# google/dynamic-video-depth

Hardware: AMD Instinct MI355X
Metric: train iters/s (depth+sceneflow step) at 384x672, 48 pairs; warp+loss HBM GB/s (higher is better)
Workload: dtype f32 (storage and accumulation fp32; conv / MLP contractions on v_mfma_f32_32x32x16_f16: every fp32 operand, scaled by a power of two from its tensor's max, is split into two fp16 terms (22 bits) and a product is three partial products; <= 4e-6 of max|y| against float64, the bound the 3-term bf16 / 6

## Files before the change

dynamic-video-depth_amd/dvd_hip/_lib.py:

```python
import ctypes
import os
import threading

from . import build as _build

c_float_p = ctypes.c_void_p
c_size_t = ctypes.c_size_t
c_int = ctypes.c_int
c_float = ctypes.c_float
c_void_p = ctypes.c_void_p

DVD_OK, DVD_EINVAL, DVD_EHIP, DVD_ENOSPC = 0, -1, -2, -3
ABI_VERSION = 8


class Cameras(ctypes.Structure):
    _fields_ = [(n, c_void_p) for n in ('R_1', 'R_2', 'R_1_T', 'R_2_T', 't_1', 't_2', 'K', 'K_inv')]


class WarpCfg(ctypes.Structure):
    _fields_ = [('B', c_int), ('H', c_int), ('W', c_int), ('midas_mask', c_int), ('crit_l2', c_int),
                ('disp_mode', c_int), ('loss_on_sf', c_int), ('flow_mul', c_float), ('disp_mul', c_float)]


# ... 161 lines not shown
    'dvd_gscale_end': (c_int, [c_void_p, c_void_p]),
    'dvd_cast_scale_f32': (c_int, [c_void_p, c_int, c_void_p, c_longlong, c_void_p, c_void_p]),
    'dvd_maxpool3s2_fwd': (c_int, [c_void_p, c_void_p, c_int, c_void_p, c_longlong, c_int, c_int, c_void_p]),
    'dvd_maxpool3s2_bwd': (c_int, [c_void_p, c_int, c_void_p, c_void_p, c_void_p, c_longlong, c_int, c_int, c_void_p]),
    'dvd_adam_step_guarded': (c_int, [c_void_p, c_void_p, c_float, c_void_p, c_void_p, c_void_p, c_void_p, c_longlong, c_float,
                                      c_float, c_float, c_float, c_int, c_void_p, c_void_p]),
    'dvd_sgd_step': (c_int, [c_void_p, c_void_p, c_float, c_void_p, c_void_p, c_void_p, c_longlong, c_float, c_float, c_float,
                             c_float, c_int, c_void_p]),
    'dvd_sgd_step_guarded': (c_int, [c_void_p, c_void_p, c_float, c_void_p, c_void_p, c_void_p, c_longlong, c_float, c_float,
                                     c_float, c_float, c_int, c_void_p, c_void_p]),
    'dvd_gather_pairs': (c_int, [ctypes.POINTER(GatherItem), c_int, c_void_p, c_int, c_void_p]),
    'dvd_store_gather': (c_int, [ctypes.POINTER(StoreItem), c_int, c_void_p, c_longlong, c_int, c_void_p]),
    'dvd_union_gather': (c_int, [c_void_p] * 5 + [c_int, c_int, c_longlong, c_void_p]),
    'dvd_union_scatter': (c_int, [c_void_p] * 5 + [c_int, c_int, c_longlong, c_void_p]),
    'dvd_union_reduce': (c_int, [c_void_p] * 5 + [c_int, c_int, c_longlong, c_void_p]),
}

_lock = threading.Lock()
_lib = None


def library_path():
    return os.environ.get('DVD_HIP_LIB') or _build.lib_path()


def load():
    global _lib
    if _lib is not None:
        return _lib
    import torch
# ... 29 lines not shown
```

dynamic-video-depth_amd/dvd_hip/conv.py:

```python
import ctypes
import os as _os
import weakref

import torch
import torch.nn.functional as F
from torch import nn

from . import _lib
from .ops import _p, _stream, _workspace, amax_of, chansum, known_amax, new_scalar, set_amax

AB = {k: False for k in ('gconv32', 'no_xwgrad3', 'no_alias', 'no_maskfuse', 'no_s2', 'rowsum')}
for _k in filter(None, _os.environ.get('DVD_AB', '').split(',')):
    if _k not in AB:
        raise RuntimeError('DVD_AB: unknown switch %r (known: %s)' % (_k, ', '.join(sorted(AB))))
    AB[_k] = True


ACT_DTYPES = (torch.float32, torch.float16)
GRAD_SCALE = {'state': None}


def set_grad_scale_state(state):
    GRAD_SCALE['state'] = state

# ... 948 lines not shown
        _lib.check(getattr(lib, family + '_h')(_p(x), _p(gy), _p(_gs(1)), *tail), family + '_h')
    elif family == 'dvd_xwgrad':
        _lib.check(lib.dvd_xwgrad(_p(x), _p(gy), *tail), family)
    elif family == 'dvd_xwgrad1s':
        _lib.check(lib.dvd_xwgrad1s_rowsum(_p(x), _p(x_amax), _p(gy), _p(g_amax), _p(gw), _p(rowsum), *tail[1:]),
                   'dvd_xwgrad1s_rowsum')
    else:
        _lib.check(getattr(lib, family)(_p(x), _p(x_amax), _p(gy), _p(g_amax), *tail), family)
    return gw


class _XConvBn(torch.autograd.Function):

    @staticmethod
    def forward(ctx, x, x_amax, weight, cbias, gamma, beta, mean, var, eps, residual, relu, groups, alias=False, in_site=None,
                out_site=None):
        ctx.set_materialize_grads(False)
        ctx.in_site = in_site if (in_site is not None and not AB['no_maskfuse']) else None
        ctx.out_site = out_site if relu else None
        x = x.contiguous()
        if residual is not None:
            residual = residual.contiguous()
        Cout, _, KS, _ = weight.shape
        y_amax, amax_slot = _fwd_amax(ctx, x)
        y = _xconv_run(x, xconv_packed(weight, False, groups), Cout, KS, bias=cbias, residual=residual, relu_out=relu,
                       groups=groups, bn=(gamma, beta, mean, var, eps), x_amax=x_amax, y_amax=amax_slot)
        ctx.save_for_backward(x, y if relu else None, gamma, mean, var, cbias, x_amax)
        ctx.wparam = weight
        ctx.cfg = (float(eps), bool(relu), residual is not None, groups)
        if alias:
            return y, y_amax, x
        return y, y_amax

    @staticmethod
    def backward(ctx, gy, _g_amax, g_alias=None):
        x, y, gamma, mean, var, cbias, x_amax = ctx.saved_tensors
        weight = ctx.wparam
        eps, relu, has_res, groups = ctx.cfg
        if gy is None:
            return (g_alias,) + (None,) * 14
        gy = gy.contiguous()
        Cout, Cing, KS, _ = weight.shape
        N, _, H, W = gy.shape
        need = ctx.needs_input_grad
        lib = _lib.load()
        dbeta = torch.empty(Cout, device=gy.device, dtype=torch.float32)
        premasked = relu and ctx.out_site is not None and ctx.out_site.is_exactly(gy) and not AB['no_maskfuse']
        mask = relu and not premasked
        need_w = need[2] or (gamma is not None and need[4]) or (cbias is not None and need[3])
        grouped3 = KS == 3 and groups > 1
        wgrad_sums = (relu and need_w and gy.dtype == torch.float32 and (grouped3 or wgrad_reports_rowsum(weight.shape, groups)) and
                      lib.dvd_xwgrad_rowsum_in_kernel(N, Cing * groups, Cout, H, W, KS, groups) == 1)
        no_pass = premasked and wgrad_sums and ctx.out_site.amax is not None
        if relu:
            STATS['sites_no_pass' if (no_pass and AB['rowsum']) else ('sites_premasked' if premasked else 'sites_masked')] += 1
        g = torch.empty_like(gy) if mask else gy
        h16 = _is16(gy)
        if no_pass:
            g_amax = ctx.out_site.amax
        else:
            ws = _workspace(lib.dvd_bnrelu_bwd_workspace_bytes(N, Cout, H * W), gy.device)
            g_amax = _gs(3) if h16 else new_scalar(gy.device)
            _lib.check(lib.dvd_bnrelu_bwd_t(_p(gy), _p(y) if mask else None, None, _p(var), _p(mean), _p(var), eps, None,
                                            _p(g) if mask else None, None, None if wgrad_sums else _p(dbeta), _p(ws),
                                            ctypes.c_size_t(ws.numel()),
                                            int(h16), _p(_gs(1)) if h16 else None, N, Cout, H * W, int(mask), _p(g_amax),
                                            _stream()), 'dvd_bnrelu_bwd')
        gx = gw = gcb = gg = None
        if need[0]:
            gx = _xconv_bwd_data(ctx, g, g_amax, weight, groups, x if ctx.in_site is not None else None, g_alias,
                                 bn_scale=(gamma, var, eps))
        elif g_alias is not None:
            gx = g_alias
        if need_w:
            if wgrad_sums and grouped3:
                gw = xconv_wgrad3_rowsum(x, g, weight.shape, groups, x_amax, g_amax, dbeta)
            else:
                gw = xconv_wgrad(x, g, weight.shape, False, groups, x_amax=x_amax, g_amax=g_amax, rowsum=dbeta if wgrad_sums else None)
            gg = torch.empty_like(gamma) if gamma is not None else None
            gcb = torch.empty_like(cbias) if cbias is not None else None
            _lib.check(lib.dvd_convbn_finalize(_p(weight.detach()), _p(gw), _p(dbeta), _p(gamma), _p(mean), _p(var), eps,
                                               _p(cbias), Cout, Cing * KS * KS, _p(gg), _p(gcb), _stream()),
                       'dvd_convbn_finalize')
        return (gx, None, gw, gcb, gg, (dbeta if need[5] else None), None, None, None, (g if has_res else None), None, None, None,
                None, None)


def conv_bn_act(conv, bn, x, residual=None, relu=True, alias=False):
    if x.is_cuda and x.dtype in ACT_DTYPES and not bn.training and bn.track_running_stats and isinstance(conv, nn.Conv2d):
        xin = None
        if xconv_supported(conv, x):
            xin = x
        elif xconv_strided_1x1_supported(conv, x):
            xin = _subsample(x, conv.stride[0])
        if xin is not None:
            gamma, beta = (bn.weight, bn.bias) if bn.affine else (None, None)
            x_amax = None if _is16(xin) else amax_of(xin)
            in_site = getattr(xin, '_dvd_site', None)
            out_site = _Site() if relu else None
            out = _XConvBn.apply(xin, x_amax, conv.weight, conv.bias, gamma, beta, bn.running_mean, bn.running_var, bn.eps,
                                 residual, relu, conv.groups, bool(alias and xin is x and not AB['no_alias']), in_site, out_site)
            out[0]._dvd_site = out_site
            y = set_amax(out[0], out[1])
            if len(out) == 3:
                return y, set_amax(out[2], x_amax)
            return (y, x) if alias else y
    y = bn_eval_relu(bn, conv(x), residual=residual, relu=relu)
    return (y, x) if alias else y


def xconv_supported(conv, x):
    k = conv.kernel_size
    return (x.is_cuda and x.dtype in ACT_DTYPES and conv.weight.dtype == torch.float32 and
            (conv.groups == 1 or (k[0] == 3 and conv.in_channels // conv.groups >= 32)) and
            k[0] == k[1] and k[0] % 2 == 1 and k[0] <= 11 and tuple(conv.stride) == (1, 1) and
            tuple(conv.dilation) == (1, 1) and tuple(conv.padding) == (k[0] // 2, k[0] // 2) and
            conv.padding_mode == 'zeros')


def xconv_strided_1x1_supported(conv, x):
    return (x.is_cuda and x.dtype in ACT_DTYPES and conv.weight.dtype == torch.float32 and conv.kernel_size == (1, 1) and
# ... 34 lines not shown
```

dynamic-video-depth_amd/dvd_hip/csrc/gconv.hip:

```cpp

#include "dvd_io.h"

namespace dvd {

constexpr int kCPG = 8;
constexpr int kWT_H = 8;

template <bool TRANSPOSED, class T, int TW, int TH>
__global__ __launch_bounds__(256) void gconv3x3_c8_kernel(const T* __restrict__ in, const float* __restrict__ w,
                                                          T* __restrict__ out, int C, int H, int W, int tiles_x) {
  typedef float v2f __attribute__((ext_vector_type(2)));
  typedef float v4f __attribute__((ext_vector_type(4)));
  constexpr int IW = TW + 2 + 2;
  constexpr int IH = TH + 2;
  constexpr int NSX = TW / 4;
  static_assert(TW % 4 == 0 && NSX * TH <= 256, "one thread per strip");
  __shared__ __attribute__((aligned(16))) float s_in[kCPG][IH][IW];
  const int tile = blockIdx.x, g = blockIdx.y, n = blockIdx.z;
  const int ty = tile / tiles_x, tx = tile - ty * tiles_x;
  const int x0 = tx * TW, y0 = ty * TH;
  const size_t plane = (size_t)H * W;
  const T* inb = in + ((size_t)n * C + (size_t)g * kCPG) * plane;
  T* outb = out + ((size_t)n * C + (size_t)g * kCPG) * plane;
  if ((W & 3) == 0) {
    constexpr int kQ = kCPG * IH * NSX, kU = (kQ + 255) / 256;
    float4 v[kU];
#pragma unroll
    for (int u = 0; u < kU; ++u) {
      const int i = threadIdx.x + u * 256;
      const int row = i / NSX, q = i - row * NSX, c = row / IH, yy = row - c * IH;
      const int gy = y0 + yy - 1, gx = x0 + q * 4;
      v[u] = (i < kQ && gy >= 0 && gy < H && gx < W) ? ld4(inb + (size_t)c * plane + (size_t)gy * W + gx)
                                                      : make_float4(0.0f, 0.0f, 0.0f, 0.0f);
    }
    constexpr int kE = kCPG * IH * 2, kUE = (kE + 255) / 256;
    float e[kUE];
#pragma unroll
    for (int u = 0; u < kUE; ++u) {
      const int i = threadIdx.x + u * 256;
      const int row = i >> 1, c = row / IH, yy = row - c * IH;
      const int gy = y0 + yy - 1, gx = (i & 1) ? x0 + TW : x0 - 1;
      e[u] = (i < kE && gy >= 0 && gy < H && gx >= 0 && gx < W) ? ldf(inb + (size_t)c * plane + (size_t)gy * W + gx) : 0.0f;
    }
#pragma unroll
    for (int u = 0; u < kU; ++u) {
      const int i = threadIdx.x + u * 256;
      if (i < kQ) {
        const int row = i / NSX, q = i - row * NSX;
        float* d = &s_in[0][0][0] + row * IW + 1 + q * 4;
        d[0] = v[u].x; d[1] = v[u].y; d[2] = v[u].z; d[3] = v[u].w;
      }
    }
#pragma unroll
    for (int u = 0; u < kUE; ++u) {
      const int i = threadIdx.x + u * 256;
      if (i < kE) (&s_in[0][0][0])[(i >> 1) * IW + ((i & 1) ? TW + 1 : 0)] = e[u];
    }
  } else {
    constexpr int kU = 8, kRow = TW + 2, kTot = kCPG * IH * kRow;
    for (int i0 = threadIdx.x; i0 < kTot; i0 += 256 * kU) {
      float v[kU];
#pragma unroll
      for (int u = 0; u < kU; ++u) {
        const int i = i0 + u * 256;
        const int c = i / (IH * kRow), r = i - c * (IH * kRow), yy = r / kRow, xx = r - yy * kRow;
        const int gy = y0 + yy - 1, gx = x0 + xx - 1;
        v[u] = (i < kTot && gy >= 0 && gy < H && gx >= 0 && gx < W) ? ldf(inb + (size_t)c * plane + (size_t)gy * W + gx) : 0.0f;
      }
#pragma unroll
      for (int u = 0; u < kU; ++u) {
        const int i = i0 + u * 256;
        if (i < kTot) {
          const int c = i / (IH * kRow), r = i - c * (IH * kRow), yy = r / kRow, xx = r - yy * kRow;
          s_in[c][yy][xx] = v[u];
        }
      }
    }
  }
  __syncthreads();
  if (threadIdx.x >= NSX * TH) return;
  const int sy = threadIdx.x / NSX, sx = threadIdx.x - sy * NSX;
  v2f acc[kCPG][2];
#pragma unroll
  for (int d = 0; d < kCPG; ++d) acc[d][0] = acc[d][1] = (v2f){0.0f, 0.0f};
  const float* wg = w + (size_t)g * (kCPG * kCPG * 9);
#pragma unroll 1
  for (int s = 0; s < kCPG; ++s) {
#pragma unroll
    for (int ky = 0; ky < 3; ++ky) {
      const float* row = &s_in[s][sy + ky][sx * 4];
      const v4f a = *reinterpret_cast<const v4f*>(row);
      const v2f b = *reinterpret_cast<const v2f*>(row + 4);
      const v2f xp[3][2] = {{{a.x, a.y}, {a.z, a.w}}, {{a.y, a.z}, {a.w, b.x}}, {{a.z, a.w}, {b.x, b.y}}};
#pragma unroll
      for (int kx = 0; kx < 3; ++kx) {
#pragma unroll
        for (int d = 0; d < kCPG; ++d) {
          const float wv = !TRANSPOSED ? wg[(d * kCPG + s) * 9 + ky * 3 + kx] : wg[(s * kCPG + d) * 9 + (2 - ky) * 3 + (2 - kx)];
          acc[d][0] = __builtin_elementwise_fma(xp[kx][0], (v2f){wv, wv}, acc[d][0]);
          acc[d][1] = __builtin_elementwise_fma(xp[kx][1], (v2f){wv, wv}, acc[d][1]);
        }
      }
    }
  }
  const int oy = y0 + sy, ox = x0 + sx * 4;
  if (oy < H && ox < W) {
    const bool vec = ((W & 3) == 0) && (ox + 3 < W);
#pragma unroll
    for (int d = 0; d < kCPG; ++d) {
      T* dst = outb + (size_t)d * plane + (size_t)oy * W + ox;
      const float o[4] = {acc[d][0].x, acc[d][0].y, acc[d][1].x, acc[d][1].y};
      if (vec) {
        st4(dst, make_float4(o[0], o[1], o[2], o[3]));
      } else {
#pragma unroll
        for (int j = 0; j < 4; ++j)
          if (ox + j < W) stf(dst + j, o[j]);
      }
    }
  }
}

template <bool TRANSPOSED>
static void launch_c8(const void* in, const float* w, void* out, int f16, int N, int C, int H, int W, hipStream_t stream) {
  if (W % 84 == 0) {
    const int tx = W / 84, ty = (H + 11) / 12;
    DVD_DISPATCH_T(f16, hipLaunchKernelGGL((gconv3x3_c8_kernel<TRANSPOSED, T, 84, 12>), dim3(tx * ty, C / kCPG, N), dim3(256), 0,
                                           stream, static_cast<const T*>(in), w, static_cast<T*>(out), C, H, W, tx));
  } else {
    const int tx = (W + 63) / 64, ty = (H + 15) / 16;
    DVD_DISPATCH_T(f16, hipLaunchKernelGGL((gconv3x3_c8_kernel<TRANSPOSED, T, 64, 16>), dim3(tx * ty, C / kCPG, N), dim3(256), 0,
                                           stream, static_cast<const T*>(in), w, static_cast<T*>(out), C, H, W, tx));
  }
}

template <class T, int TW>
__global__ __launch_bounds__(256) void gconv3x3_c8_wgrad_kernel(const T* __restrict__ x, const T* __restrict__ gy,
                                                                float* __restrict__ partial, int C, int H, int W,
                                                                int tiles_x, int G) {
  typedef float v2f __attribute__((ext_vector_type(2)));
  typedef float v4f __attribute__((ext_vector_type(4)));
  constexpr int IW = 68;
  constexpr int IH = kWT_H + 2;
  constexpr int XP = IH * IW + 4;
  constexpr int GW2 = 144;
  constexpr int GP2 = kWT_H * GW2 + 4;
  constexpr int kRedBytes = kWT_H * 32 * 18 * 4, kXBytes = kCPG * XP * 4;
  __shared__ __attribute__((aligned(16))) float s_x[(kRedBytes > kXBytes ? kRedBytes : kXBytes) / 4];
  __shared__ __attribute__((aligned(16))) float s_g[(kCPG / 2) * GP2];
  const int band = blockIdx.x, g = blockIdx.y, n = blockIdx.z;
  const int y0 = band * kWT_H;
  const size_t plane = (size_t)H * W;
  const T* xb = x + ((size_t)n * C + (size_t)g * kCPG) * plane;
  const T* gb = gy + ((size_t)n * C + (size_t)g * kCPG) * plane;
  const bool vec = (W & 3) == 0;

  constexpr int NQ = TW / 4;
  constexpr int kXQ = kCPG * IH * NQ, kUX = (kXQ + 255) / 256;
  constexpr int kXE = kCPG * IH * 2;
  constexpr int kGQ = (kCPG / 2) * kWT_H * NQ, kUG = (kGQ + 255) / 256;
  float4 xv[kUX], g0[kUG], g1[kUG];
  float xe;
  auto fetch = [&](int x0) {
    const float4 z = make_float4(0.0f, 0.0f, 0.0f, 0.0f);
#pragma unroll
    for (int u = 0; u < kUX; ++u) {
      const int i = threadIdx.x + u * 256;
      const int row = i / NQ, q = i - row * NQ, c = row / IH, yy = row - c * IH;
      const int py = y0 + yy - 1, px = x0 + q * 4;
      xv[u] = (i < kXQ && py >= 0 && py < H && px < W) ? ld4(xb + (size_t)c * plane + (size_t)py * W + px) : z;
    }
    {
      const int i = threadIdx.x, row = i >> 1, c = row / IH, yy = row - c * IH;
      const int py = y0 + yy - 1, px = (i & 1) ? x0 + TW : x0 - 1;
      xe = (i < kXE && py >= 0 && py < H && px >= 0 && px < W) ? ldf(xb + (size_t)c * plane + (size_t)py * W + px) : 0.0f;
    }
#pragma unroll
// ... 17 lines not shown
        d[0] = xv[u].x; d[1] = xv[u].y; d[2] = xv[u].z; d[3] = xv[u].w;
      }
    }
    if (threadIdx.x < kXE) {
      const int row = threadIdx.x >> 1, c = row / IH, yy = row - c * IH;
      s_x[c * XP + yy * IW + ((threadIdx.x & 1) ? TW + 1 : 0)] = xe;
    }
#pragma unroll
    for (int u = 0; u < kUG; ++u) {
      const int i = threadIdx.x + u * 256;
      if (i < kGQ) {
        const int row = i / NQ, q = i - row * NQ, cp = row / kWT_H, yy = row - cp * kWT_H;
        v4f* d = reinterpret_cast<v4f*>(&s_g[cp * GP2 + yy * GW2 + q * 8]);
        d[0] = (v4f){g0[u].x, g1[u].x, g0[u].y, g1[u].y};
        d[1] = (v4f){g0[u].z, g1[u].z, g0[u].w, g1[u].w};
      }
    }
  };
  auto stage_scalar = [&](int x0) {
    constexpr int kU = 8, kRow = TW + 2, kTot = kCPG * IH * kRow;
    for (int i0 = threadIdx.x; i0 < kTot; i0 += 256 * kU) {
      float v[kU];
#pragma unroll
      for (int u = 0; u < kU; ++u) {
        const int i = i0 + u * 256;
        const int c = i / (IH * kRow), r = i - c * (IH * kRow), yy = r / kRow, xx = r - yy * kRow;
        const int py = y0 + yy - 1, px = x0 + xx - 1;
        v[u] = (i < kTot && py >= 0 && py < H && px >= 0 && px < W) ? ldf(xb + (size_t)c * plane + (size_t)py * W + px) : 0.0f;
      }
#pragma unroll
// ... 9 lines not shown
    for (int i0 = threadIdx.x; i0 < kTotG; i0 += 256 * kU) {
      float v[kU];
#pragma unroll
      for (int u = 0; u < kU; ++u) {
        const int i = i0 + u * 256;
        const int c = i / (kWT_H * TW), r = i - c * (kWT_H * TW), yy = r / TW, xx = r - yy * TW;
        const int py = y0 + yy, px = x0 + xx;
        v[u] = (i < kTotG && py < H && px < W) ? ldf(gb + (size_t)c * plane + (size_t)py * W + px) : 0.0f;
      }
#pragma unroll
      for (int u = 0; u < kU; ++u) {
        const int i = i0 + u * 256;
        if (i < kTotG) {
          const int c = i / (kWT_H * TW), r = i - c * (kWT_H * TW), yy = r / TW, xx = r - yy * TW;
          s_g[(c >> 1) * GP2 + yy * GW2 + xx * 2 + (c & 1)] = v[u];
        }
      }
    }
  };

  const int lane = threadIdx.x & 63, wave = threadIdx.x >> 6;
  const int r = wave * 2 + (lane >> 5), cp = (lane >> 3) & 3, ci = lane & 7;
  v2f acc[9];
#pragma unroll
  for (int t = 0; t < 9; ++t) acc[t] = (v2f){0.0f, 0.0f};
  const float* grow = &s_g[cp * GP2 + r * GW2];
  const float* xrow = &s_x[ci * XP + r * IW];
  if (vec) fetch(0);
  for (int tx = 0; tx < tiles_x; ++tx) {
    if (vec) put(); else stage_scalar(tx * TW);
// ... 20 lines not shown
    __syncthreads();
  }
  float* s_red = s_x;
#pragma unroll
  for (int t = 0; t < 9; ++t) *reinterpret_cast<v2f*>(&s_red[((r * 32 + cp * 8 + ci) * 9 + t) * 2]) = acc[t];
  __syncthreads();
  float* dst = partial + ((size_t)(n * gridDim.x + band) * G + g) * 576;
  for (int i = threadIdx.x; i < 576; i += 256) {
    const int co = i / 72, rem = i - co * 72, ci2 = rem / 9, t = rem - ci2 * 9;
    const int src = (((co >> 1) * 8 + ci2) * 9 + t) * 2 + (co & 1);
    float sum = s_red[src];
#pragma unroll
    for (int rr = 1; rr < kWT_H; ++rr) sum += s_red[rr * 576 + src];
    dst[i] = sum;
  }
}

__global__ __launch_bounds__(256) void gconv_wgrad_reduce_kernel(const float* __restrict__ partial, float* __restrict__ gw,
                                                                 int n_records, int n_weights, int accumulate,
                                                                 const float* __restrict__ out_scale) {
  __shared__ float s_part[3][64];
  const int lane = threadIdx.x & 63, cls = threadIdx.x >> 6;
  const int i = blockIdx.x * 64 + lane;
  const bool live = i < n_weights;
  float s = 0.0f;
  if (live) {
    const int n4 = n_records & ~3;
    const float* p = partial + i;
#pragma unroll 8
    for (int r = cls; r < n4; r += 4) s += p[(size_t)r * n_weights];
    if (cls == 0)
      for (int r = n4; r < n_records; ++r) s += p[(size_t)r * n_weights];
  }
  if (cls > 0) s_part[cls - 1][lane] = s;
  __syncthreads();
  if (cls == 0 && live) {
    const float t = ((s + s_part[0][lane]) + (s_part[1][lane] + s_part[2][lane])) * (out_scale ? out_scale[0] : 1.0f);
    gw[i] = accumulate ? gw[i] + t : t;
// ... 35 lines not shown

int dvd_gconv3x3_c8_bwd_data_t(const void* gy, const float* w, void* gx, int f16, int N, int C, int H, int W,
                               dvd_stream_t stream) {
  if (int e = dvd::check_shape(N, C, H, W)) return e;
  DVD_REQUIRE(gy && w && gx, "gconv bwd_data: null pointer");
  dvd::bytes_add(DVD_BYTES_GCONV, 2.0 * N * C * (double)H * W * (f16 ? 2 : 4));
  dvd::launch_c8<true>(gy, w, gx, f16, N, C, H, W, static_cast<hipStream_t>(stream));
  DVD_LAUNCH_OK();
  return DVD_OK;
}

size_t dvd_gconv3x3_c8_wgrad_workspace_bytes(int N, int C, int H, int W) {
  if (N <= 0 || C <= 0 || H <= 0 || W <= 0 || C % dvd::kCPG) return 0;
  const size_t tiles = (size_t)((H + dvd::kWT_H - 1) / dvd::kWT_H);
  return tiles * N * (size_t)C * dvd::kCPG * 9 * sizeof(float);
}

int dvd_gconv3x3_c8_bwd_weight_t(const void* x, const void* gy, float* gw, int accumulate, void* workspace,
                                 size_t workspace_bytes, int f16, const float* out_scale, int N, int C, int H, int W,
                                 dvd_stream_t stream) {
  if (int e = dvd::check_shape(N, C, H, W)) return e;
  DVD_REQUIRE(x && gy && gw && workspace, "gconv bwd_weight: null pointer");
  dvd::bytes_add(DVD_BYTES_GCONV, 2.0 * N * C * (double)H * W * (f16 ? 2 : 4));
  const size_t need = dvd_gconv3x3_c8_wgrad_workspace_bytes(N, C, H, W);
  if (workspace_bytes < need) {
    dvd::set_error("gconv bwd_weight: workspace %zu < %zu bytes", workspace_bytes, need);
    return DVD_ENOSPC;
  }
  const int tw = dvd::wgrad_tile_w(W);
  const int tx = (W + tw - 1) / tw, bands = (H + dvd::kWT_H - 1) / dvd::kWT_H;
  const int G = C / dvd::kCPG;
  if (tw == 56) {
    DVD_DISPATCH_T(f16, hipLaunchKernelGGL((dvd::gconv3x3_c8_wgrad_kernel<T, 56>), dim3(bands, G, N), dim3(256), 0,
                                           static_cast<hipStream_t>(stream), static_cast<const T*>(x),
                                           static_cast<const T*>(gy), static_cast<float*>(workspace), C, H, W, tx, G));
  } else {
    DVD_DISPATCH_T(f16, hipLaunchKernelGGL((dvd::gconv3x3_c8_wgrad_kernel<T, 64>), dim3(bands, G, N), dim3(256), 0,
                                           static_cast<hipStream_t>(stream), static_cast<const T*>(x),
                                           static_cast<const T*>(gy), static_cast<float*>(workspace), C, H, W, tx, G));
  }
  DVD_LAUNCH_OK();
  const int n_weights = C * dvd::kCPG * 9;
  hipLaunchKernelGGL(dvd::gconv_wgrad_reduce_kernel, dim3((n_weights + 63) / 64), dim3(256), 0,
                     static_cast<hipStream_t>(stream), static_cast<const float*>(workspace), gw, bands * N, n_weights,
                     accumulate, out_scale);
  DVD_LAUNCH_OK();
  return DVD_OK;
}

}
```

include/dvd_hip.h:

```cpp
#ifndef DVD_HIP_H
#define DVD_HIP_H

#include <stddef.h>
#include <stdint.h>

#ifdef __cplusplus
extern "C" {
#endif

#define DVD_ABI_VERSION 8

typedef void* dvd_stream_t;

typedef enum dvd_status {
  DVD_OK = 0,
  DVD_EINVAL = -1,
  DVD_EHIP = -2,
  DVD_ENOSPC = -3
} dvd_status;

int dvd_abi_version(void);
const char* dvd_last_error(void);
int dvd_device_cu_count(void);

// ... 128 lines not shown
                          const dvd_cameras* cams, const dvd_surfaces* g_surfaces, float* g_depth_1, float* g_depth_2,
                          float* g_sflow_1_2, int B, int H, int W, dvd_stream_t stream);

int dvd_flow_warp_fwd(const float* buffer, const float* flow_1_2, float* out, int B, int C, int H, int W,
                      dvd_stream_t stream);
int dvd_flow_warp_bwd(const float* g_out, const float* flow_1_2, float* g_buffer, int B, int C, int H, int W,
                      dvd_stream_t stream);

int dvd_gconv3x3_c8_fwd(const float* x, const float* w, float* y, int N, int C, int H, int W,
                        dvd_stream_t stream);
int dvd_gconv3x3_c8_bwd_data(const float* gy, const float* w, float* gx, int N, int C, int H, int W,
                             dvd_stream_t stream);
size_t dvd_gconv3x3_c8_wgrad_workspace_bytes(int N, int C, int H, int W);
int dvd_gconv3x3_c8_bwd_weight(const float* x, const float* gy, float* gw, int accumulate, void* workspace,
                               size_t workspace_bytes, int N, int C, int H, int W, dvd_stream_t stream);

size_t dvd_gconv3x3_c32_workspace_bytes(int N, int C, int H, int W);
int dvd_gconv3x3_c32_fwd(const float* x, const float* w, float* y, void* workspace, size_t workspace_bytes, int N,
                         int C, int H, int W, dvd_stream_t stream);
int dvd_gconv3x3_c32_bwd_data(const float* gy, const float* w, float* gx, void* workspace, size_t workspace_bytes,
                              int N, int C, int H, int W, dvd_stream_t stream);
int dvd_gconv3x3_c32_bwd_weight(const float* x, const float* gy, float* gw, int accumulate, void* workspace,
                                size_t workspace_bytes, int N, int C, int H, int W, dvd_stream_t stream);

int dvd_bnrelu_fwd(const float* x, const float* residual, const float* gamma, const float* beta, const float* mean,
                   const float* var, float eps, float* y, int N, int C, int HW, int relu, dvd_stream_t stream);
size_t dvd_bnrelu_bwd_workspace_bytes(int N, int C, int HW);
int dvd_bnrelu_bwd(const float* gy, const float* y, const float* x, const float* gamma, const float* mean,
                   const float* var, float eps, float* gx, float* g_residual, float* g_gamma, float* g_beta,
                   void* workspace, size_t workspace_bytes, int N, int C, int HW, int relu, float* g_amax, dvd_stream_t stream);
// ... 173 lines not shown
```

Measured before the change: 1.614.

## Fuse BN+ReLU into grouped 3x3 conv sites and add stride-2 XConvBn path

Adds a fused grouped 3x3 (8 channels per group) conv path that applies eval-mode BN scale/shift, ReLU and amax tracking in the conv epilogue. Its backward folds the BN scale and input ReLU mask into the data-gradient kernel and computes the per-channel gradient sums inside the weight-gradient kernel. Also routes stride-2 and 16-channel-per-group conv+BN sites through the existing fused XConvBn kernels, subsampling the gradient for weight grads. This is meant to remove separate BN/ReLU passes and the extra activation reads and writes they cost. The price is more kernel variants, and the new dispatch only covers fp32 inputs.

```diff
diff --git a/dynamic-video-depth_amd/dvd_hip/_lib.py b/dynamic-video-depth_amd/dvd_hip/_lib.py
--- a/dynamic-video-depth_amd/dvd_hip/_lib.py
+++ b/dynamic-video-depth_amd/dvd_hip/_lib.py
@@ -199,6 +199,11 @@
     'dvd_union_gather': (c_int, [c_void_p] * 5 + [c_int, c_int, c_longlong, c_void_p]),
     'dvd_union_scatter': (c_int, [c_void_p] * 5 + [c_int, c_int, c_longlong, c_void_p]),
     'dvd_union_reduce': (c_int, [c_void_p] * 5 + [c_int, c_int, c_longlong, c_void_p]),
+    'dvd_gconv3x3_c8_bn_fwd': (c_int, [c_void_p] * 6 + [c_float, c_void_p, c_void_p, c_int, c_int, c_int, c_int, c_void_p]),
+    'dvd_gconv3x3_c8_bn_bwd_data': (c_int, [c_void_p] * 4 + [c_float, c_void_p, c_void_p, c_void_p, c_int, c_int, c_int, c_int,
+                                            c_void_p]),
+    'dvd_gconv3x3_c8_bn_wgrad_workspace_bytes': (c_size_t, [c_int, c_int, c_int, c_int]),
+    'dvd_gconv3x3_c8_bn_bwd_weight': (c_int, [c_void_p] * 5 + [c_size_t, c_int, c_int, c_int, c_int, c_void_p]),
 }
 
 _lock = threading.Lock()
diff --git a/dynamic-video-depth_amd/dvd_hip/conv.py b/dynamic-video-depth_amd/dvd_hip/conv.py
--- a/dynamic-video-depth_amd/dvd_hip/conv.py
+++ b/dynamic-video-depth_amd/dvd_hip/conv.py
@@ -986,7 +986,7 @@
 
     @staticmethod
     def forward(ctx, x, x_amax, weight, cbias, gamma, beta, mean, var, eps, residual, relu, groups, alias=False, in_site=None,
-                out_site=None):
+                out_site=None, stride=1):
         ctx.set_materialize_grads(False)
         ctx.in_site = in_site if (in_site is not None and not AB['no_maskfuse']) else None
         ctx.out_site = out_site if relu else None
@@ -996,10 +996,11 @@
         Cout, _, KS, _ = weight.shape
         y_amax, amax_slot = _fwd_amax(ctx, x)
         y = _xconv_run(x, xconv_packed(weight, False, groups), Cout, KS, bias=cbias, residual=residual, relu_out=relu,
-                       groups=groups, bn=(gamma, beta, mean, var, eps), x_amax=x_amax, y_amax=amax_slot)
+                       groups=groups, bn=(gamma, beta, mean, var, eps), x_amax=x_amax, y_amax=amax_slot,
+                       **({'stride': 2} if stride == 2 else {}))
         ctx.save_for_backward(x, y if relu else None, gamma, mean, var, cbias, x_amax)
         ctx.wparam = weight
-        ctx.cfg = (float(eps), bool(relu), residual is not None, groups)
+        ctx.cfg = (float(eps), bool(relu), residual is not None, groups, int(stride))
         if alias:
             return y, y_amax, x
         return y, y_amax
@@ -1008,9 +1009,9 @@
     def backward(ctx, gy, _g_amax, g_alias=None):
         x, y, gamma, mean, var, cbias, x_amax = ctx.saved_tensors
         weight = ctx.wparam
-        eps, relu, has_res, groups = ctx.cfg
+        eps, relu, has_res, groups, stride = ctx.cfg
         if gy is None:
-            return (g_alias,) + (None,) * 14
+            return (g_alias,) + (None,) * 15
         gy = gy.contiguous()
         Cout, Cing, KS, _ = weight.shape
         N, _, H, W = gy.shape
@@ -1021,8 +1022,9 @@
         mask = relu and not premasked
         need_w = need[2] or (gamma is not None and need[4]) or (cbias is not None and need[3])
         grouped3 = KS == 3 and groups > 1
+        wH, wW = (x.shape[2], x.shape[3]) if stride == 2 else (H, W)
         wgrad_sums = (relu and need_w and gy.dtype == torch.float32 and (grouped3 or wgrad_reports_rowsum(weight.shape, groups)) and
-                      lib.dvd_xwgrad_rowsum_in_kernel(N, Cing * groups, Cout, H, W, KS, groups) == 1)
+                      lib.dvd_xwgrad_rowsum_in_kernel(N, Cing * groups, Cout, wH, wW, KS, groups) == 1)
         no_pass = premasked and wgrad_sums and ctx.out_site.amax is not None
         if relu:
             STATS['sites_no_pass' if (no_pass and AB['rowsum']) else ('sites_premasked' if premasked else 'sites_masked')] += 1
@@ -1040,22 +1042,107 @@
                                             _stream()), 'dvd_bnrelu_bwd')
         gx = gw = gcb = gg = None
         if need[0]:
+            strided = dict(stride=-2, out_hw=(x.shape[2], x.shape[3])) if stride == 2 else {}
             gx = _xconv_bwd_data(ctx, g, g_amax, weight, groups, x if ctx.in_site is not None else None, g_alias,
-                                 bn_scale=(gamma, var, eps))
+                                 bn_scale=(gamma, var, eps), **strided)
         elif g_alias is not None:
             gx = g_alias
         if need_w:
+            gf = g
+            if stride == 2:
+                gf = torch.empty(N, Cout, wH, wW, device=g.device, dtype=g.dtype)
+                _lib.check(lib.dvd_subsample2_bwd(_p(g), _p(gf), int(h16), N * Cout, wH, wW, _stream()), 'dvd_subsample2_bwd')
             if wgrad_sums and grouped3:
-                gw = xconv_wgrad3_rowsum(x, g, weight.shape, groups, x_amax, g_amax, dbeta)
+                gw = xconv_wgrad3_rowsum(x, gf, weight.shape, groups, x_amax, g_amax, dbeta)
             else:
-                gw = xconv_wgrad(x, g, weight.shape, False, groups, x_amax=x_amax, g_amax=g_amax, rowsum=dbeta if wgrad_sums else None)
+                gw = xconv_wgrad(x, gf, weight.shape, False, groups, x_amax=x_amax, g_amax=g_amax, rowsum=dbeta if wgrad_sums else None)
             gg = torch.empty_like(gamma) if gamma is not None else None
             gcb = torch.empty_like(cbias) if cbias is not None else None
             _lib.check(lib.dvd_convbn_finalize(_p(weight.detach()), _p(gw), _p(dbeta), _p(gamma), _p(mean), _p(var), eps,
                                                _p(cbias), Cout, Cing * KS * KS, _p(gg), _p(gcb), _stream()),
                        'dvd_convbn_finalize')
         return (gx, None, gw, gcb, gg, (dbeta if need[5] else None), None, None, None, (g if has_res else None), None, None, None,
-                None, None)
+                None, None, None)
+
+
+class _GConvBn(torch.autograd.Function):
+
+    @staticmethod
+    def forward(ctx, x, weight, gamma, beta, mean, var, eps, in_site, out_site):
+        ctx.set_materialize_grads(False)
+        ctx.in_site = in_site if (in_site is not None and not AB['no_maskfuse']) else None
+        ctx.out_site = out_site
+        x = x.contiguous()
+        N, C, H, W = x.shape
+        y = torch.empty_like(x)
+        y_amax = new_scalar(x.device)
+        ctx.mark_non_differentiable(y_amax)
+        _lib.check(_lib.load().dvd_gconv3x3_c8_bn_fwd(_p(x), _p(weight), _p(gamma), _p(beta), _p(mean), _p(var), float(eps), _p(y),
+                                                      _p(y_amax), N, C, H, W, _stream()), 'dvd_gconv3x3_c8_bn_fwd')
+        ctx.save_for_backward(x, y, weight, gamma, mean, var)
+        ctx.eps = float(eps)
+        return y, y_amax
+
+    @staticmethod
+    def backward(ctx, gy, _g_amax):
+        x, y, weight, gamma, mean, var = ctx.saved_tensors
+        if gy is None:
+            return (None,) * 9
+        gy = gy.contiguous()
+        N, C, H, W = x.shape
+        eps = ctx.eps
+        need = ctx.needs_input_grad
+        lib = _lib.load()
+        premasked = ctx.out_site is not None and ctx.out_site.is_exactly(gy) and not AB['no_maskfuse']
+        STATS['sites_premasked' if premasked else 'sites_masked'] += 1
+        g = gy
+        if not premasked:
+            g = torch.empty_like(gy)
+            ws = _workspace(lib.dvd_bnrelu_bwd_workspace_bytes(N, C, H * W), gy.device)
+            _lib.check(lib.dvd_bnrelu_bwd_t(_p(gy), _p(y), None, _p(var), _p(mean), _p(var), eps, None, _p(g), None, None, _p(ws),
+                                            ctypes.c_size_t(ws.numel()), 0, None, N, C, H * W, 1, None, _stream()), 'dvd_bnrelu_bwd')
+        gx = gw = gg = dbeta = None
+        if need[0]:
+            gx = torch.empty_like(x)
+            gx_amax = new_scalar(gy.device)
+            _lib.check(lib.dvd_gconv3x3_c8_bn_bwd_data(_p(g), _p(weight), _p(gamma), _p(var), eps,
+                                                       _p(x) if ctx.in_site is not None else None, _p(gx), _p(gx_amax), N, C, H, W,
+                                                       _stream()), 'dvd_gconv3x3_c8_bn_bwd_data')
+            set_amax(gx, gx_amax)
+            if ctx.in_site is not None:
+                ctx.in_site.wrote(gx, gx_amax)
+        if need[1] or need[2] or need[3]:
+            gw = torch.empty_like(weight)
+            dbeta = torch.empty(C, device=gy.device, dtype=torch.float32)
+            ws = _workspace(lib.dvd_gconv3x3_c8_bn_wgrad_workspace_bytes(N, C, H, W), gy.device)
+            _lib.check(lib.dvd_gconv3x3_c8_bn_bwd_weight(_p(x), _p(g), _p(gw), _p(dbeta), _p(ws), ctypes.c_size_t(ws.numel()), N, C,
+                                                         H, W, _stream()), 'dvd_gconv3x3_c8_bn_bwd_weight')
+            gg = torch.empty_like(gamma)
+            _lib.check(lib.dvd_convbn_finalize(_p(weight), _p(gw), _p(dbeta), _p(gamma), _p(mean), _p(var), eps, None, C, 72,
+                                               _p(gg), None, _stream()), 'dvd_convbn_finalize')
+        return gx, gw, gg, (dbeta if need[3] else None), None, None, None, None, None
+
+
+def _conv2_site_kind(conv, bn, x, residual, relu):
+    if not (x.dtype == torch.float32 and relu and residual is None and bn.affine and conv.bias is None and
+            conv.weight.dtype == torch.float32 and conv.kernel_size == (3, 3) and tuple(conv.padding) == (1, 1) and
+            tuple(conv.dilation) == (1, 1) and conv.padding_mode == 'zeros' and x.dim() == 4):
+        return None
+    cpg, st = conv.in_channels // conv.groups, tuple(conv.stride)
+    if conv.in_channels != conv.out_channels and conv.groups > 1:
+        return None
+    if st == (1, 1):
+        if cpg == 8 and conv.groups > 1:
+            return 'c8'
+        if cpg == 16 and conv.groups > 1 and conv.in_channels % 32 == 0 and not AB['gconv32']:
+            return 'c16'
+        return None
+    if st == (2, 2) and not AB['no_s2']:
+        if cpg == 16 and conv.groups > 1:
+            return 's2' if (conv.in_channels % 32 == 0 and not AB['gconv32']) else None
+        if xconv_s2_supported(x, conv.weight, conv.groups):
+            return 's2'
+    return None
 
 
 def conv_bn_act(conv, bn, x, residual=None, relu=True, alias=False):
@@ -1077,6 +1164,21 @@
             if len(out) == 3:
                 return y, set_amax(out[2], x_amax)
             return (y, x) if alias else y
+        kind = _conv2_site_kind(conv, bn, x, residual, relu)
+        if kind is not None:
+            in_site, out_site = getattr(x, '_dvd_site', None), _Site()
+            stats = (bn.running_mean, bn.running_var, bn.eps)
+            if kind == 'c8':
+                y, y_amax = _GConvBn.apply(x, conv.weight, bn.weight, bn.bias, *stats, in_site, out_site)
+            else:
+                w, groups = conv.weight, conv.groups
+                if w.shape[1] == 16:
+                    w, groups = _pair_groups_of_16(w), groups // 2
+                y, y_amax = _XConvBn.apply(x, amax_of(x), w, None, bn.weight, bn.bias, *stats, None, True, groups, False, in_site,
+                                           out_site, 2 if kind == 's2' else 1)
+            y._dvd_site = out_site
+            y = set_amax(y, y_amax)
+            return (y, x) if alias else y
     y = bn_eval_relu(bn, conv(x), residual=residual, relu=relu)
     return (y, x) if alias else y
 
diff --git a/dynamic-video-depth_amd/dvd_hip/csrc/gconv.hip b/dynamic-video-depth_amd/dvd_hip/csrc/gconv.hip
--- a/dynamic-video-depth_amd/dvd_hip/csrc/gconv.hip
+++ b/dynamic-video-depth_amd/dvd_hip/csrc/gconv.hip
@@ -6,9 +6,19 @@
 constexpr int kCPG = 8;
 constexpr int kWT_H = 8;
 
-template <bool TRANSPOSED, class T, int TW, int TH>
+struct GSite {
+  const float* gamma;
+  const float* beta;
+  const float* mean;
+  const float* var;
+  float eps;
+  const void* mask;
+  float* amax;
+};
+
+template <bool TRANSPOSED, class T, int TW, int TH, bool SITE>
 __global__ __launch_bounds__(256) void gconv3x3_c8_kernel(const T* __restrict__ in, const float* __restrict__ w,
-                                                          T* __restrict__ out, int C, int H, int W, int tiles_x) {
+                                                          T* __restrict__ out, int C, int H, int W, int tiles_x, GSite site) {
   typedef float v2f __attribute__((ext_vector_type(2)));
   typedef float v4f __attribute__((ext_vector_type(4)));
   constexpr int IW = TW + 2 + 2;
@@ -16,12 +26,22 @@
   constexpr int NSX = TW / 4;
   static_assert(TW % 4 == 0 && NSX * TH <= 256, "one thread per strip");
   __shared__ __attribute__((aligned(16))) float s_in[kCPG][IH][IW];
+  __shared__ float s_bn[SITE ? 2 : 1][kCPG];
   const int tile = blockIdx.x, g = blockIdx.y, n = blockIdx.z;
   const int ty = tile / tiles_x, tx = tile - ty * tiles_x;
   const int x0 = tx * TW, y0 = ty * TH;
   const size_t plane = (size_t)H * W;
   const T* inb = in + ((size_t)n * C + (size_t)g * kCPG) * plane;
   T* outb = out + ((size_t)n * C + (size_t)g * kCPG) * plane;
+  auto bn_setup = [&]() {
+    if (threadIdx.x < kCPG) {
+      const int c = g * kCPG + threadIdx.x;
+      const float s = site.gamma[c] / sqrtf(site.var[c] + site.eps);
+      s_bn[0][threadIdx.x] = s;
+      if (!TRANSPOSED) s_bn[SITE ? 1 : 0][threadIdx.x] = site.beta[c] - site.mean[c] * s;
+    }
+    if (TRANSPOSED) __syncthreads();
+  };
   if ((W & 3) == 0) {
     constexpr int kQ = kCPG * IH * NSX, kU = (kQ + 255) / 256;
     float4 v[kU];
@@ -42,22 +62,28 @@
       const int gy = y0 + yy - 1, gx = (i & 1) ? x0 + TW : x0 - 1;
       e[u] = (i < kE && gy >= 0 && gy < H && gx >= 0 && gx < W) ? ldf(inb + (size_t)c * plane + (size_t)gy * W + gx) : 0.0f;
     }
+    if (SITE) bn_setup();
 #pragma unroll
     for (int u = 0; u < kU; ++u) {
       const int i = threadIdx.x + u * 256;
       if (i < kQ) {
         const int row = i / NSX, q = i - row * NSX;
         float* d = &s_in[0][0][0] + row * IW + 1 + q * 4;
+        if (SITE && TRANSPOSED) {
+          const float sc = s_bn[0][row / IH];
+          v[u].x *= sc; v[u].y *= sc; v[u].z *= sc; v[u].w *= sc;
+        }
         d[0] = v[u].x; d[1] = v[u].y; d[2] = v[u].z; d[3] = v[u].w;
       }
     }
 #pragma unroll
     for (int u = 0; u < kUE; ++u) {
       const int i = threadIdx.x + u * 256;
-      if (i < kE) (&s_in[0][0][0])[(i >> 1) * IW + ((i & 1) ? TW + 1 : 0)] = e[u];
+      if (i < kE) (&s_in[0][0][0])[(i >> 1) * IW + ((i & 1) ? TW + 1 : 0)] = (SITE && TRANSPOSED) ? e[u] * s_bn[0][(i >> 1) / IH] : e[u];
     }
   } else {
     constexpr int kU = 8, kRow = TW + 2, kTot = kCPG * IH * kRow;
+    if (SITE) bn_setup();
     for (int i0 = threadIdx.x; i0 < kTot; i0 += 256 * kU) {
       float v[kU];
 #pragma unroll
@@ -72,13 +98,16 @@
         const int i = i0 + u * 256;
         if (i < kTot) {
           const int c = i / (IH * kRow), r = i - c * (IH * kRow), yy = r / kRow, xx = r - yy * kRow;
-          s_in[c][yy][xx] = v[u];
+          s_in[c][yy][xx] = (SITE && TRANSPOSED) ? v[u] * s_bn[0][c] : v[u];
         }
       }
     }
   }
   __syncthreads();
-  if (threadIdx.x >= NSX * TH) return;
+  const bool active = threadIdx.x < NSX * TH;
+  if (!SITE && !active) return;
+  float m = 0.0f;
+  if (active) {
   const int sy = threadIdx.x / NSX, sx = threadIdx.x - sy * NSX;
   v2f acc[kCPG][2];
 #pragma unroll
@@ -106,38 +135,88 @@
   const int oy = y0 + sy, ox = x0 + sx * 4;
   if (oy < H && ox < W) {
     const bool vec = ((W & 3) == 0) && (ox + 3 < W);
+    const T* maskb = (SITE && TRANSPOSED) ? static_cast<const T*>(site.mask) : nullptr;
+    if (maskb) maskb += ((size_t)n * C + (size_t)g * kCPG) * plane;
 #pragma unroll
     for (int d = 0; d < kCPG; ++d) {
-      T* dst = outb + (size_t)d * plane + (size_t)oy * W + ox;
-      const float o[4] = {acc[d][0].x, acc[d][0].y, acc[d][1].x, acc[d][1].y};
+      const size_t off = (size_t)d * plane + (size_t)oy * W + ox;
+      T* dst = outb + off;
+      float o[4] = {acc[d][0].x, acc[d][0].y, acc[d][1].x, acc[d][1].y};
+      if (SITE && !TRANSPOSED) {
+        const float bs = s_bn[0][d], bb = s_bn[SITE ? 1 : 0][d];
+#pragma unroll
+        for (int j = 0; j < 4; ++j) o[j] = fmaxf(__builtin_fmaf(o[j], bs, bb), 0.0f);
+      }
       if (vec) {
+        if (maskb) {
+          const float4 k = ld4(maskb + off);
+          o[0] = k.x > 0.0f ? o[0] : 0.0f;
+          o[1] = k.y > 0.0f ? o[1] : 0.0f;
+          o[2] = k.z > 0.0f ? o[2] : 0.0f;
+          o[3] = k.w > 0.0f ? o[3] : 0.0f;
+        }
         st4(dst, make_float4(o[0], o[1], o[2], o[3]));
+        if (SITE) m = amax_acc(amax_acc(amax_acc(amax_acc(m, o[0]), o[1]), o[2]), o[3]);
       } else {
 #pragma unroll
         for (int j = 0; j < 4; ++j)
-          if (ox + j < W) stf(dst + j, o[j]);
-      }
+          if (ox + j < W) {
+            if (maskb) o[j] = ldf(maskb + off + j) > 0.0f ? o[j] : 0.0f;
+            stf(dst + j, o[j]);
+            if (SITE) m = amax_acc(m, o[j]);
+          }
+      }
+    }
+  }
+  }
+  if (SITE && site.amax) {
+    float* s_m = &s_bn[0][0];
+#pragma unroll
+    for (int off = kWave / 2; off > 0; off >>= 1) m = fmaxf(m, __shfl_down(m, off, kWave));
+    __syncthreads();
+    if ((threadIdx.x & 63) == 0) s_m[threadIdx.x >> 6] = m;
+    __syncthreads();
+    if (threadIdx.x == 0) {
+      m = fmaxf(fmaxf(s_m[0], s_m[1]), fmaxf(s_m[2], s_m[3]));
+      unsigned* p = reinterpret_cast<unsigned*>(site.amax);
+      if (m > 0.0f && __float_as_uint(m) > __hip_atomic_load(p, __ATOMIC_RELAXED, __HIP_MEMORY_SCOPE_AGENT))
+        atomicMax(p, __float_as_uint(m));
     }
   }
 }
 
 template <bool TRANSPOSED>
 static void launch_c8(const void* in, const float* w, void* out, int f16, int N, int C, int H, int W, hipStream_t stream) {
+  const GSite none = {};
   if (W % 84 == 0) {
     const int tx = W / 84, ty = (H + 11) / 12;
-    DVD_DISPATCH_T(f16, hipLaunchKernelGGL((gconv3x3_c8_kernel<TRANSPOSED, T, 84, 12>), dim3(tx * ty, C / kCPG, N), dim3(256), 0,
-                                           stream, static_cast<const T*>(in), w, static_cast<T*>(out), C, H, W, tx));
+    DVD_DISPATCH_T(f16, hipLaunchKernelGGL((gconv3x3_c8_kernel<TRANSPOSED, T, 84, 12, false>), dim3(tx * ty, C / kCPG, N), dim3(256),
+                                           0, stream, static_cast<const T*>(in), w, static_cast<T*>(out), C, H, W, tx, none));
   } else {
     const int tx = (W + 63) / 64, ty = (H + 15) / 16;
-    DVD_DISPATCH_T(f16, hipLaunchKernelGGL((gconv3x3_c8_kernel<TRANSPOSED, T, 64, 16>), dim3(tx * ty, C / kCPG, N), dim3(256), 0,
-                                           stream, static_cast<const T*>(in), w, static_cast<T*>(out), C, H, W, tx));
-  }
-}
-
-template <class T, int TW>
+    DVD_DISPATCH_T(f16, hipLaunchKernelGGL((gconv3x3_c8_kernel<TRANSPOSED, T, 64, 16, false>), dim3(tx * ty, C / kCPG, N), dim3(256),
+                                           0, stream, static_cast<const T*>(in), w, static_cast<T*>(out), C, H, W, tx, none));
+  }
+}
+
+template <bool TRANSPOSED>
+static void launch_c8_site(const float* in, const float* w, float* out, const GSite& site, int N, int C, int H, int W,
+                           hipStream_t stream) {
+  if (W % 84 == 0) {
+    const int tx = W / 84, ty = (H + 11) / 12;
+    hipLaunchKernelGGL((gconv3x3_c8_kernel<TRANSPOSED, float, 84, 12, true>), dim3(tx * ty, C / kCPG, N), dim3(256), 0, stream, in, w,
+                       out, C, H, W, tx, site);
+  } else {
+    const int tx = (W + 63) / 64, ty = (H + 15) / 16;
+    hipLaunchKernelGGL((gconv3x3_c8_kernel<TRANSPOSED, float, 64, 16, true>), dim3(tx * ty, C / kCPG, N), dim3(256), 0, stream, in, w,
+                       out, C, H, W, tx, site);
+  }
+}
+
+template <class T, int TW, bool SUMS>
 __global__ __launch_bounds__(256) void gconv3x3_c8_wgrad_kernel(const T* __restrict__ x, const T* __restrict__ gy,
                                                                 float* __restrict__ partial, int C, int H, int W,
-                                                                int tiles_x, int G) {
+                                                                int tiles_x, int G, float* __restrict__ sums) {
   typedef float v2f __attribute__((ext_vector_type(2)));
   typedef float v4f __attribute__((ext_vector_type(4)));
   constexpr int IW = 68;
@@ -161,6 +240,12 @@
   constexpr int kGQ = (kCPG / 2) * kWT_H * NQ, kUG = (kGQ + 255) / 256;
   float4 xv[kUX], g0[kUG], g1[kUG];
   float xe;
+  float rs[kCPG];
+#pragma unroll
+  for (int c = 0; c < kCPG; ++c) rs[c] = 0.0f;
+  float rq0[kUG], rq1[kUG];
+#pragma unroll
+  for (int u = 0; u < kUG; ++u) rq0[u] = rq1[u] = 0.0f;
   auto fetch = [&](int x0) {
     const float4 z = make_float4(0.0f, 0.0f, 0.0f, 0.0f);
 #pragma unroll
@@ -208,6 +293,10 @@
         v4f* d = reinterpret_cast<v4f*>(&s_g[cp * GP2 + yy * GW2 + q * 8]);
         d[0] = (v4f){g0[u].x, g1[u].x, g0[u].y, g1[u].y};
         d[1] = (v4f){g0[u].z, g1[u].z, g0[u].w, g1[u].w};
+        if (SUMS) {
+          rq0[u] += (g0[u].x + g0[u].y) + (g0[u].z + g0[u].w);
+          rq1[u] += (g1[u].x + g1[u].y) + (g1[u].z + g1[u].w);
+        }
       }
     }
   };
@@ -247,6 +336,10 @@
         if (i < kTotG) {
           const int c = i / (kWT_H * TW), r = i - c * (kWT_H * TW), yy = r / TW, xx = r - yy * TW;
           s_g[(c >> 1) * GP2 + yy * GW2 + xx * 2 + (c & 1)] = v[u];
+          if (SUMS) {
+#pragma unroll
+            for (int k = 0; k < kCPG; ++k) rs[k] += (c == k) ? v[u] : 0.0f;
+          }
         }
       }
     }
@@ -297,14 +390,63 @@
     for (int rr = 1; rr < kWT_H; ++rr) sum += s_red[rr * 576 + src];
     dst[i] = sum;
   }
+  if (SUMS) {
+    if (vec) {
+#pragma unroll
+      for (int u = 0; u < kUG; ++u) {
+        const int cpu = (threadIdx.x + u * 256) / (NQ * kWT_H);
+#pragma unroll
+        for (int k = 0; k < kCPG; ++k) rs[k] += (2 * cpu == k) ? rq0[u] : ((2 * cpu + 1 == k) ? rq1[u] : 0.0f);
+      }
+    }
+    float* s_sum = s_g;
+#pragma unroll
+    for (int k = 0; k < kCPG; ++k) s_sum[k * 256 + threadIdx.x] = rs[k];
+    __syncthreads();
+    double part = 0.0;
+    if (threadIdx.x < 64) {
+      const float* q = s_sum + (threadIdx.x >> 3) * 256 + (threadIdx.x & 7) * 32;
+#pragma unroll 8
+      for (int j = 0; j < 32; ++j) part += (double)q[j];
+    }
+    __syncthreads();
+    double* s_part = reinterpret_cast<double*>(s_sum);
+    if (threadIdx.x < 64) s_part[threadIdx.x] = part;
+    __syncthreads();
+    if (threadIdx.x < kCPG) {
+      const double* q = s_part + threadIdx.x * 8;
+      double sum = q[0];
+#pragma unroll
+      for (int j = 1; j < 8; ++j) sum += q[j];
+      sums[((size_t)(n * gridDim.x + band) * G + g) * kCPG + threadIdx.x] = (float)sum;
+    }
+  }
 }
 
 __global__ __launch_bounds__(256) void gconv_wgrad_reduce_kernel(const float* __restrict__ partial, float* __restrict__ gw,
                                                                  int n_records, int n_weights, int accumulate,
-                                                                 const float* __restrict__ out_scale) {
+                                                                 const float* __restrict__ out_scale, int blocks1,
+                                                                 const float* __restrict__ partial2, float* __restrict__ out2,
+                                                                 int n2) {
   __shared__ float s_part[3][64];
   const int lane = threadIdx.x & 63, cls = threadIdx.x >> 6;
-  const int i = blockIdx.x * 64 + lane;
+  if ((int)blockIdx.x >= blocks1) {
+    __shared__ double s_partd[3][64];
+    const int c = (blockIdx.x - blocks1) * 64 + lane;
+    double d = 0.0;
+    if (c < n2) {
+      const int n4 = n_records & ~3;
+      for (int r = cls; r < n4; r += 4) d += (double)partial2[(size_t)r * n2 + c];
+      if (cls == 0)
+        for (int r = n4; r < n_records; ++r) d += (double)partial2[(size_t)r * n2 + c];
+    }
+    if (cls > 0) s_partd[cls - 1][lane] = d;
+    __syncthreads();
+    if (cls == 0 && c < n2) out2[c] = (float)((d + s_partd[0][lane]) + (s_partd[1][lane] + s_partd[2][lane]));
+    return;
+  }
+  const int blk = blockIdx.x;
+  const int i = blk * 64 + lane;
   const bool live = i < n_weights;
   float s = 0.0f;
   if (live) {
@@ -370,6 +512,37 @@
   if (N <= 0 || C <= 0 || H <= 0 || W <= 0 || C % dvd::kCPG) return 0;
   const size_t tiles = (size_t)((H + dvd::kWT_H - 1) / dvd::kWT_H);
   return tiles * N * (size_t)C * dvd::kCPG * 9 * sizeof(float);
+}
+
+static int gconv_c8_wgrad(const void* x, const void* gy, float* gw, int accumulate, void* workspace, int f16,
+                          const float* out_scale, float* chansum, int N, int C, int H, int W, dvd_stream_t stream) {
+  const int tw = dvd::wgrad_tile_w(W);
+  const int tx = (W + tw - 1) / tw, bands = (H + dvd::kWT_H - 1) / dvd::kWT_H;
+  const int G = C / dvd::kCPG;
+  const int n_weights = C * dvd::kCPG * 9;
+  float* partial = static_cast<float*>(workspace);
+  float* sums = partial + (size_t)bands * N * n_weights;
+  hipStream_t s = static_cast<hipStream_t>(stream);
+  if (chansum) {
+    if (tw == 56)
+      hipLaunchKernelGGL((dvd::gconv3x3_c8_wgrad_kernel<float, 56, true>), dim3(bands, G, N), dim3(256), 0, s,
+                         static_cast<const float*>(x), static_cast<const float*>(gy), partial, C, H, W, tx, G, sums);
+    else
+      hipLaunchKernelGGL((dvd::gconv3x3_c8_wgrad_kernel<float, 64, true>), dim3(bands, G, N), dim3(256), 0, s,
+                         static_cast<const float*>(x), static_cast<const float*>(gy), partial, C, H, W, tx, G, sums);
+  } else if (tw == 56) {
+    DVD_DISPATCH_T(f16, hipLaunchKernelGGL((dvd::gconv3x3_c8_wgrad_kernel<T, 56, false>), dim3(bands, G, N), dim3(256), 0, s,
+                                           static_cast<const T*>(x), static_cast<const T*>(gy), partial, C, H, W, tx, G, nullptr));
+  } else {
+    DVD_DISPATCH_T(f16, hipLaunchKernelGGL((dvd::gconv3x3_c8_wgrad_kernel<T, 64, false>), dim3(bands, G, N), dim3(256), 0, s,
+                                           static_cast<const T*>(x), static_cast<const T*>(gy), partial, C, H, W, tx, G, nullptr));
+  }
+  DVD_LAUNCH_OK();
+  const int blocks1 = (n_weights + 63) / 64, blocks2 = chansum ? (C + 63) / 64 : 0;
+  hipLaunchKernelGGL(dvd::gconv_wgrad_reduce_kernel, dim3(blocks1 + blocks2), dim3(256), 0, s, partial, gw, bands * N, n_weights,
+                     accumulate, out_scale, blocks1, sums, chansum, C);
+  DVD_LAUNCH_OK();
+  return DVD_OK;
 }
 
 int dvd_gconv3x3_c8_bwd_weight_t(const void* x, const void* gy, float* gw, int accumulate, void* workspace,
@@ -383,25 +556,51 @@
     dvd::set_error("gconv bwd_weight: workspace %zu < %zu bytes", workspace_bytes, need);
     return DVD_ENOSPC;
   }
-  const int tw = dvd::wgrad_tile_w(W);
-  const int tx = (W + tw - 1) / tw, bands = (H + dvd::kWT_H - 1) / dvd::kWT_H;
-  const int G = C / dvd::kCPG;
-  if (tw == 56) {
-    DVD_DISPATCH_T(f16, hipLaunchKernelGGL((dvd::gconv3x3_c8_wgrad_kernel<T, 56>), dim3(bands, G, N), dim3(256), 0,
-                                           static_cast<hipStream_t>(stream), static_cast<const T*>(x),
-                                           static_cast<const T*>(gy), static_cast<float*>(workspace), C, H, W, tx, G));
-  } else {
-    DVD_DISPATCH_T(f16, hipLaunchKernelGGL((dvd::gconv3x3_c8_wgrad_kernel<T, 64>), dim3(bands, G, N), dim3(256), 0,
-                                           static_cast<hipStream_t>(stream), static_cast<const T*>(x),
-                                           static_cast<const T*>(gy), static_cast<float*>(workspace), C, H, W, tx, G));
-  }
-  DVD_LAUNCH_OK();
-  const int n_weights = C * dvd::kCPG * 9;
-  hipLaunchKernelGGL(dvd::gconv_wgrad_reduce_kernel, dim3((n_weights + 63) / 64), dim3(256), 0,
-                     static_cast<hipStream_t>(stream), static_cast<const float*>(workspace), gw, bands * N, n_weights,
-                     accumulate, out_scale);
+  return gconv_c8_wgrad(x, gy, gw, accumulate, workspace, f16, out_scale, nullptr, N, C, H, W, stream);
+}
+
+int dvd_gconv3x3_c8_bn_fwd(const float* x, const float* w, const float* gamma, const float* beta, const float* mean,
+                           const float* var, float eps, float* y, float* y_amax, int N, int C, int H, int W,
+                           dvd_stream_t stream) {
+  if (int e = dvd::check_shape(N, C, H, W)) return e;
+  DVD_REQUIRE(x && w && y && gamma && beta && mean && var, "gconv bn fwd: null pointer");
+  dvd::bytes_add(DVD_BYTES_GCONV, 2.0 * N * C * (double)H * W * 4);
+  const dvd::GSite site = {gamma, beta, mean, var, eps, nullptr, y_amax};
+  dvd::launch_c8_site<false>(x, w, y, site, N, C, H, W, static_cast<hipStream_t>(stream));
   DVD_LAUNCH_OK();
   return DVD_OK;
 }
 
-}
+int dvd_gconv3x3_c8_bn_bwd_data(const float* g, const float* w, const float* gamma, const float* var, float eps,
+                                const float* mask_src, float* gx, float* gx_amax, int N, int C, int H, int W,
+                                dvd_stream_t stream) {
+  if (int e = dvd::check_shape(N, C, H, W)) return e;
+  DVD_REQUIRE(g && w && gx && gamma && var, "gconv bn bwd_data: null pointer");
+  dvd::bytes_add(DVD_BYTES_GCONV, (mask_src ? 3.0 : 2.0) * N * C * (double)H * W * 4);
+  const dvd::GSite site = {gamma, nullptr, nullptr, var, eps, mask_src, gx_amax};
+  dvd::launch_c8_site<true>(g, w, gx, site, N, C, H, W, static_cast<hipStream_t>(stream));
+  DVD_LAUNCH_OK();
+  return DVD_OK;
+}
+
+size_t dvd_gconv3x3_c8_bn_wgrad_workspace_bytes(int N, int C, int H, int W) {
+  const size_t base = dvd_gconv3x3_c8_wgrad_workspace_bytes(N, C, H, W);
+  if (base == 0) return 0;
+  const size_t bands = (size_t)((H + dvd::kWT_H - 1) / dvd::kWT_H);
+  return base + bands * N * (size_t)C * sizeof(float);
+}
+
+int dvd_gconv3x3_c8_bn_bwd_weight(const float* x, const float* g, float* gw, float* g_chansum, void* workspace,
+                                  size_t workspace_bytes, int N, int C, int H, int W, dvd_stream_t stream) {
+  if (int e = dvd::check_shape(N, C, H, W)) return e;
+  DVD_REQUIRE(x && g && gw && g_chansum && workspace, "gconv bn bwd_weight: null pointer");
+  dvd::bytes_add(DVD_BYTES_GCONV, 2.0 * N * C * (double)H * W * 4);
+  const size_t need = dvd_gconv3x3_c8_bn_wgrad_workspace_bytes(N, C, H, W);
+  if (workspace_bytes < need) {
+    dvd::set_error("gconv bn bwd_weight: workspace %zu < %zu bytes", workspace_bytes, need);
+    return DVD_ENOSPC;
+  }
+  return gconv_c8_wgrad(x, g, gw, 0, workspace, 0, nullptr, g_chansum, N, C, H, W, stream);
+}
+
+}
diff --git a/include/dvd_hip.h b/include/dvd_hip.h
--- a/include/dvd_hip.h
+++ b/include/dvd_hip.h
@@ -166,6 +166,16 @@
 size_t dvd_gconv3x3_c8_wgrad_workspace_bytes(int N, int C, int H, int W);
 int dvd_gconv3x3_c8_bwd_weight(const float* x, const float* gy, float* gw, int accumulate, void* workspace,
                                size_t workspace_bytes, int N, int C, int H, int W, dvd_stream_t stream);
+
+int dvd_gconv3x3_c8_bn_fwd(const float* x, const float* w, const float* gamma, const float* beta, const float* mean,
+                           const float* var, float eps, float* y, float* y_amax, int N, int C, int H, int W,
+                           dvd_stream_t stream);
+int dvd_gconv3x3_c8_bn_bwd_data(const float* g, const float* w, const float* gamma, const float* var, float eps,
+                                const float* mask_src, float* gx, float* gx_amax, int N, int C, int H, int W,
+                                dvd_stream_t stream);
+size_t dvd_gconv3x3_c8_bn_wgrad_workspace_bytes(int N, int C, int H, int W);
+int dvd_gconv3x3_c8_bn_bwd_weight(const float* x, const float* g, float* gw, float* g_chansum, void* workspace,
+                                  size_t workspace_bytes, int N, int C, int H, int W, dvd_stream_t stream);
 
 size_t dvd_gconv3x3_c32_workspace_bytes(int N, int C, int H, int W);
 int dvd_gconv3x3_c32_fwd(const float* x, const float* w, float* y, void* workspace, size_t workspace_bytes, int N,
```

Result: faster. 1.638, median of 6 (+1.5%).
